# octavian-ganea/equidock_public

Hardware: AMD Instinct MI355X
Metric: protein-pairs/sec (fwd+bwd) per IEGMN stack (higher is better)
Workload: dtype f32; 1 GPU; B: DB5.5-sized batch of 8 pairs x (200,200) residues, k=10, 8-layer IEGMN hdim 64, 50 heads, fp32; pairs_per_gpu=8, nodes_per_gpu=3200, edges_per_gpu=32000, layers=8, parallelism=dp1, weights=PyTorch default init (seed 0), ROT key/query x40 (SURVEY.md section 8c), svd_guard_pairs=0, launch_mode=hipGraph replay

## Files before the change

### equidock_public_amd/_lib.py

```python
import ctypes as C
import os

import torch

HERE = os.path.dirname(os.path.abspath(__file__))
LIB_PATH = os.path.join(HERE, 'libequidock_hip.so')
if os.environ.get('EQD_EXP_LIBRARY'):
    LIB_PATH = os.environ['EQD_EXP_LIBRARY']

EQD_MAX_SRC = 6
ABI_VERSION = 9
PARAMS_PER_LAYER = 19
GLOBAL_PARAMS = 5

c_float_p = C.POINTER(C.c_float)
c_int_p = C.POINTER(C.c_int32)


class EqdGraph(C.Structure):
    _fields_ = [('n_pairs', C.c_int32), ('n_lig', C.c_int32), ('n_rec', C.c_int32), ('n_nodes', C.c_int32),
                ('n_edges', C.c_int32), ('n_tiles', C.c_int32), ('n_att_items', C.c_int32), ('max_seg', C.c_int32),
                ('seg_off', C.c_void_p), ('src', C.c_void_p), ('dst', C.c_void_p), ('rowptr', C.c_void_p),
                ('csc_ptr', C.c_void_p), ('csc_eid', C.c_void_p), ('tile_node', C.c_void_p),
                ('att_items', C.c_void_p), ('res_id', C.c_void_p), ('mu_r_norm', C.c_void_p), ('he', C.c_void_p),
# ... 31 lines not shown
    _fields_ = [('X', C.c_void_p), ('xmask', C.c_void_p), ('ldx', C.c_int32), ('M', C.c_int32), ('Y', C.c_void_p),
                ('ldy', C.c_int32), ('N', C.c_int32), ('rows', C.c_int32), ('out', C.c_void_p), ('o_rs', C.c_int32),
                ('o_cs', C.c_int32), ('bias_out', C.c_void_p), ('slope', C.c_float), ('scale', C.c_float), ('bf16', C.c_int32),
                ('y_bf16', C.c_int32)]


class EqdEdgeParams(C.Structure):
    _fields_ = [('W1', C.c_void_p), ('ldw1', C.c_int32), ('d_in', C.c_int32), ('ln_g', C.c_void_p),
                ('ln_b', C.c_void_p), ('W2', C.c_void_p), ('b2', C.c_void_p), ('Wc1', C.c_void_p),
                ('bc1', C.c_void_p), ('wc2', C.c_void_p), ('bc2', C.c_void_p), ('slope', C.c_float),
                ('ln_eps', C.c_float), ('eta', C.c_float), ('use_dist', C.c_int32), ('use_he', C.c_int32),
                ('bf16', C.c_int32), ('drop_z1', C.c_void_p), ('drop_ch', C.c_void_p), ('drop_scale', C.c_float),
                ('aggr_bf16', C.c_void_p), ('xh_save', C.c_void_p), ('rstd_save', C.c_void_p), ('zpos_save', C.c_void_p)]


class EqdNodeUpdateParams(C.Structure):
    _fields_ = [('d_in', C.c_int32), ('d0', C.c_int32), ('d_out', C.c_int32), ('ld_cross', C.c_int32), ('Wn1', C.c_void_p),
                ('bn1', C.c_void_p), ('ln_g', C.c_void_p), ('ln_b', C.c_void_p), ('Wn2', C.c_void_p), ('bn2', C.c_void_p),
                ('skip_weight_h', C.c_float), ('slope', C.c_float), ('ln_eps', C.c_float), ('bf16', C.c_int32),
                ('drop_mul', C.c_void_p)]


class EqdNodeUpdateGrads(C.Structure):
    _fields_ = [('dWn1', C.c_void_p), ('dbn1', C.c_void_p), ('dln_g', C.c_void_p), ('dln_b', C.c_void_p),
                ('dWn2', C.c_void_p), ('dbn2', C.c_void_p)]


class EqdEdgeGrads(C.Structure):
    _fields_ = [('dW1', C.c_void_p), ('ldw1', C.c_int32), ('db1_unused', C.c_void_p), ('dln_g', C.c_void_p),
                ('dln_b', C.c_void_p), ('dW2', C.c_void_p), ('db2', C.c_void_p), ('dWc1', C.c_void_p),
                ('dbc1', C.c_void_p), ('dwc2', C.c_void_p), ('dbc2', C.c_void_p)]


_lib = None
_is_sim = False
profiling = False


class EquidockHipError(RuntimeError):
    pass


def _declare(lib):
    lib.eqd_abi_version.restype = C.c_int
    lib.eqd_last_error.restype = C.c_char_p
    lib.eqd_tile_edges.restype = C.c_int
    lib.eqd_is_simulator.restype = C.c_int
    lib.eqd_model_saved_bytes.restype = C.c_size_t
    lib.eqd_model_scratch_bytes.restype = C.c_size_t
    lib.eqd_atb_partial_bytes.restype = C.c_size_t
    lib.eqd_edge_message_bwd_workspace_bytes.restype = C.c_size_t
    lib.eqd_keypoint_pool_bwd_workspace_bytes.restype = C.c_size_t
    lib.eqd_clash_workspace_bytes.restype = C.c_size_t
    lib.eqd_node_update_bwd_workspace_bytes.restype = C.c_size_t
    lib.eqd_cross_attention_bwd_ds_workspace_bytes.restype = C.c_size_t
    lib.eqd_profile_name.restype = C.c_char_p
    lib.eqd_profile_us.restype = C.c_float
    lib.eqd_tunables_reload.restype = None
    for name in ('eqd_model_layer_state', 'eqd_model_lrelu_signs', 'eqd_model_head_backward', 'eqd_profile_begin', 'eqd_profile_end', 'eqd_profile_mark', 'eqd_ctx_create', 'eqd_ctx_destroy', 'eqd_model_check', 'eqd_model_forward', 'eqd_model_backward', 'eqd_linear', 'eqd_atb',
                 'eqd_edge_message_fwd', 'eqd_edge_message_bwd', 'eqd_edge_message_bwd_kernel_only',
                 'eqd_cross_attention_fwd', 'eqd_cross_attention_fwd_bf16', 'eqd_cross_attention_bwd_bf16',
                 'eqd_cross_attention_bwd', 'eqd_cross_attention_bwd_ds',
           'eqd_keypoint_pool_fwd', 'eqd_keypoint_pool_bwd', 'eqd_kabsch_fwd', 'eqd_kabsch_bwd',
                 'eqd_rigid_apply_fwd', 'eqd_rigid_apply_bwd', 'eqd_pair_losses_fwd', 'eqd_pair_losses_bwd', 'eqd_scalar_loss', 'eqd_pocket_ot_cost',
                 'eqd_pocket_ot_fwd', 'eqd_pocket_ot_bwd', 'eqd_rigid_augment', 'eqd_protein_graph_distances',
                 'eqd_protein_graph_select', 'eqd_protein_graph_edges', 'eqd_clash_iterations', 'eqd_dropout_pack_edges', 'eqd_dropout_draw',
                 'eqd_node_update_fwd', 'eqd_node_update_bwd', 'eqd_selftest_lane_exchanges'):
        getattr(lib, name).restype = C.c_int


EXPORTS = ('eqd_model_layer_state', 'eqd_model_lrelu_signs', 'eqd_model_head_backward', 'eqd_profile_begin', 'eqd_profile_end', 'eqd_profile_mark', 'eqd_profile_name', 'eqd_profile_us', 'eqd_ctx_create', 'eqd_ctx_destroy', 'eqd_abi_version', 'eqd_last_error', 'eqd_tile_edges', 'eqd_is_simulator', 'eqd_model_saved_bytes', 'eqd_model_saved_layout',
           'eqd_model_scratch_bytes', 'eqd_model_check', 'eqd_model_forward', 'eqd_model_backward', 'eqd_linear',
           'eqd_atb_partial_bytes', 'eqd_atb', 'eqd_edge_message_fwd', 'eqd_edge_message_bwd_workspace_bytes',
           'eqd_edge_message_bwd', 'eqd_edge_message_bwd_kernel_only', 'eqd_cross_attention_fwd',
           'eqd_cross_attention_bwd', 'eqd_cross_attention_bwd_ds', 'eqd_cross_attention_bwd_ds_workspace_bytes', 'eqd_cross_attention_fwd_bf16', 'eqd_cross_attention_bwd_bf16',
           'eqd_keypoint_pool_fwd', 'eqd_keypoint_pool_bwd',
           'eqd_keypoint_pool_bwd_workspace_bytes',
           'eqd_kabsch_fwd', 'eqd_kabsch_bwd', 'eqd_rigid_apply_fwd', 'eqd_rigid_apply_bwd', 'eqd_pair_losses_fwd',
           'eqd_pair_losses_bwd', 'eqd_scalar_loss', 'eqd_pocket_ot_cost', 'eqd_pocket_ot_fwd', 'eqd_pocket_ot_bwd',
           'eqd_rigid_augment', 'eqd_protein_graph_distances', 'eqd_protein_graph_select', 'eqd_protein_graph_edges',
           'eqd_clash_workspace_bytes', 'eqd_clash_iterations', 'eqd_dropout_pack_edges', 'eqd_dropout_draw',
           'eqd_tunables_reload', 'eqd_node_update_fwd', 'eqd_node_update_bwd_workspace_bytes', 'eqd_node_update_bwd',
           'eqd_selftest_lane_exchanges', 'eqd_chain_resident_proj_launches', 'eqd_selftest_node_chain_fwd', 'eqd_model_node_state',
           'eqd_chain_resident_wide_launches', 'eqd_chain_resident_wide_bwd_launches', 'eqd_selftest_node_chain_bwd_wide')


def load_library():
    global _lib, _is_sim
    if _lib is not None:
        return _lib
    if not os.path.exists(LIB_PATH):
        raise EquidockHipError(
            f"{LIB_PATH} is missing: build it with `python -m equidock_public_amd.build` (hipcc, gfx950). "
            "There is no CPU fallback for the IEGMN hot path.")
    lib = C.CDLL(LIB_PATH)
    _declare(lib)
    if lib.eqd_abi_version() != ABI_VERSION:
        raise EquidockHipError(f"ABI version mismatch: library {lib.eqd_abi_version()} != {ABI_VERSION}")
    _lib, _is_sim = lib, bool(lib.eqd_is_simulator())
    return _lib


def load_library_for_testing(path):
    global _lib, _is_sim
    lib = C.CDLL(path)
    _declare(lib)
    _lib, _is_sim = lib, bool(lib.eqd_is_simulator())
    return _lib


def unload_for_testing():
    global _lib, _is_sim
    _lib, _is_sim = None, False


tunables_generation = 0


def reload_tunables():
    global tunables_generation
    tunables_generation += 1
    if _lib is not None:
        _lib.eqd_tunables_reload()


def is_simulator():
    return _is_sim


def check(rc):
    if rc != 0:
        raise EquidockHipError(f"libequidock_hip error {rc}: {_lib.eqd_last_error().decode()}")


def require_device(t, what='tensor'):
    if _is_sim:
        if t.is_cuda:
            raise EquidockHipError(f"{what}: the host simulator only takes CPU tensors")
    elif not t.is_cuda:
        raise EquidockHipError(
            f"{what} is on {t.device}: the IEGMN hot path runs only on an MI355X through libequidock_hip.so "
            "(no CPU fallback)")
    return t


class device_guard:

    def __init__(self, device):
        self._cm = None if (_is_sim or torch.device(device).type != 'cuda') else torch.cuda.device(device)

    def __enter__(self):
        if self._cm is not None:
            self._cm.__enter__()

    def __exit__(self, *exc):
        if self._cm is not None:
            self._cm.__exit__(*exc)
        return False


def ptr(t):
    return C.c_void_p(t.data_ptr()) if t is not None else C.c_void_p(0)


def stream_ptr(device):
    if _is_sim:
        return C.c_void_p(0)
# ... 32 lines not shown
```

### equidock_public_amd/csrc/eqd_attn_fwd_inl.h

```cpp
#pragma once
#include "eqd_common.h"

#ifndef EQD_NATIVE_EXP
#define EQD_NATIVE_EXP(x) __expf(x)
#endif
__device__ __forceinline__ float bwd_exp(float x) { return EQD_NATIVE_EXP(x); }

template <int DB>
struct AttnCfg {
    enum { DS = 16 * DB + 4, KS = 4 * DB, NL = 8 * DB, TILE = 32 * (16 * DB + 4), RED = DB * 2 * 4 * 64 };
};

template <int DB, bool FAST>
struct TileRegs {
    float4 q[FAST ? 8 : 1];
    float4 qx[(FAST && DB > 4) ? 2 : 1];
    f32x4 qv[FAST ? 1 : 2 * DB];
    int nvalid;
};

template <int DB, bool FAST>
__device__ __forceinline__ void tile_load(TileRegs<DB, FAST>& R, const float* __restrict__ M, int d, int r0, int r1,
                                          int lane) {
    int nrows = r1 - r0;
// ... 191 lines not shown
#if !defined(EQD_HOSTSIM) && !defined(EQD_NO_LDS_BATCH)
        __builtin_amdgcn_sched_barrier(0);
#endif
#pragma unroll
        for (int ks = 0; ks < KS; ++ks) {
#pragma unroll
            for (int nb = 0; nb < NB; ++nb) acc[nb] = mfma4(a[ks], F[nb].v[ks], acc[nb]);
        }
    }
}
template <bool BF, int DB, int NB>
__device__ __forceinline__ void mma_r2(f32x4 (&acc)[DB][NB], const float* __restrict__ A, int g, int DS, int l15,
                                       const f32x4 (&B)[2][NB]);
template <bool BF, int DB, int NB>
__device__ __forceinline__ void mma_r(f32x4 (&acc)[DB][NB], const float* __restrict__ A, int row0, int DS, int l15,
                                      const f32x4 (&B)[NB]) {
    if constexpr (BF) {
        s16x4 b[NB];
#pragma unroll
        for (int nb = 0; nb < NB; ++nb) b[nb] = pack_bf4(B[nb][0], B[nb][1], B[nb][2], B[nb][3]);
#pragma unroll
        for (int db = 0; db < DB; ++db) {
            const s16x4 a = pack_bf4(A[row0 * DS + 16 * db + l15], A[(row0 + 1) * DS + 16 * db + l15],
                                     A[(row0 + 2) * DS + 16 * db + l15], A[(row0 + 3) * DS + 16 * db + l15]);
#pragma unroll
            for (int nb = 0; nb < NB; ++nb) acc[db][nb] = mfma_bf(a, b[nb], acc[db][nb]);
        }
    } else {
        float a[4][DB];
#pragma unroll
        for (int r = 0; r < 4; ++r)
#pragma unroll
            for (int db = 0; db < DB; ++db) a[r][db] = A[(row0 + r) * DS + 16 * db + l15];
#if !defined(EQD_HOSTSIM) && !defined(EQD_NO_LDS_BATCH)
        __builtin_amdgcn_sched_barrier(0);
#endif
#pragma unroll
        for (int r = 0; r < 4; ++r)
#pragma unroll
            for (int db = 0; db < DB; ++db) {
#pragma unroll
                for (int nb = 0; nb < NB; ++nb) acc[db][nb] = mfma4(a[r][db], B[nb][r], acc[db][nb]);
            }
    }
}
template <bool BF, int DB, int NB>
__device__ __forceinline__ void mma_r2(f32x4 (&acc)[DB][NB], const float* __restrict__ A, int g, int DS, int l15,
                                       const f32x4 (&B)[2][NB]) {
    if constexpr (BF) {
        s16x8 b[NB];
#pragma unroll
        for (int nb = 0; nb < NB; ++nb)
            b[nb] = cat_bf(pack_bf4(B[0][nb][0], B[0][nb][1], B[0][nb][2], B[0][nb][3]),
                           pack_bf4(B[1][nb][0], B[1][nb][1], B[1][nb][2], B[1][nb][3]));
#pragma unroll
        for (int db = 0; db < DB; ++db) {
            const int r0 = 4 * g, r1 = 16 + 4 * g;
            const s16x8 a = cat_bf(pack_bf4(A[r0 * DS + 16 * db + l15], A[(r0 + 1) * DS + 16 * db + l15],
                                            A[(r0 + 2) * DS + 16 * db + l15], A[(r0 + 3) * DS + 16 * db + l15]),
                                   pack_bf4(A[r1 * DS + 16 * db + l15], A[(r1 + 1) * DS + 16 * db + l15],
                                            A[(r1 + 2) * DS + 16 * db + l15], A[(r1 + 3) * DS + 16 * db + l15]));
#pragma unroll
            for (int nb = 0; nb < NB; ++nb) acc[db][nb] = mfma_bf32(a, b[nb], acc[db][nb]);
        }
    } else {
        mma_r<false, DB, NB>(acc, A, 4 * g, DS, l15, B[0]);
        mma_r<false, DB, NB>(acc, A, 16 + 4 * g, DS, l15, B[1]);
    }
}

template <int DB>
struct alignas(16) AttnFwdSmem {
    typedef AttnCfg<DB> C;
    float Qt[C::TILE];
    float Kt[EQD_WAVES][C::TILE];
    float Vt[EQD_WAVES][C::TILE];
    float sm_m[EQD_WAVES][32], sm_l[EQD_WAVES][32];
    static_assert(C::RED <= C::TILE, "merge buffer must fit a K tile");
};

__device__ __forceinline__ int att_half_item(int b) { return ((b >> 4) << 3) + (b & 7); }
__device__ __forceinline__ int att_half_of(int b) { return (b >> 3) & 1; }

template <int DB, bool FAST, int NB, bool BF = false>
__device__ __forceinline__ void attn_fwd_body(AttnFwdSmem<DB>& sm, const EqdGraph& G, int item, int half, int t, int d,
                                              const float* __restrict__ q, const float* __restrict__ k,
                                              const float* __restrict__ v, float* __restrict__ out,
                                              float* __restrict__ lse, bool group_barriers = false) {
    typedef AttnCfg<DB> C;
    constexpr int DS = C::DS, KS = C::KS;
    float* Qt = sm.Qt;
    float (*Kt)[C::TILE] = sm.Kt;
    float (*Vt)[C::TILE] = sm.Vt;
    float (*sm_m)[32] = sm.sm_m;
    float (*sm_l)[32] = sm.sm_l;
    float (*red)[C::TILE] = Kt;
    const int lane = t & 63, wave = t >> 6;
    const int l15 = lane & 15, g = lane >> 4;
    int b0 = G.att_items[item * 4 + 0], b1 = G.att_items[item * 4 + 1];
    const int o0 = G.att_items[item * 4 + 2], o1 = G.att_items[item * 4 + 3];
    if (NB == 1) {
        b0 += 16 * half;
        b1 = b1 < b0 + 16 ? b1 : b0 + 16;
    }
    if (b0 >= b1) {
        if (group_barriers) {
            static_assert(!(NB == 1) || FAST, "half blocks exist on the float4 path only");
            __syncthreads();
            __syncthreads();
        }
        return;
    }
    int rowq[NB];
    bool qv[NB];
#pragma unroll
    for (int nb = 0; nb < NB; ++nb) {
        rowq[nb] = b0 + 16 * nb + l15;
        qv[nb] = rowq[nb] < b1;
    }

    EQD_TR_WG();
    EQD_TR(0);
    TileRegs<DB, FAST> rk, rv;
    int kt = o0 + 32 * wave;
    tile_load<DB, FAST>(rk, k, d, kt, o1, lane);
    tile_load<DB, FAST>(rv, v, d, kt, o1, lane);
    if (FAST) {
        EQD_TR(1);
        block_tile_stage_fast<DB>(q, DS, b0, b1, Qt, t);
    } else {
        zero_fill(Qt, C::TILE, t, EQD_BLOCK);
        zero_fill(Kt[wave], C::TILE, lane, 64);
        zero_fill(Vt[wave], C::TILE, lane, 64);
        __syncthreads();
        EQD_TR(1);
        block_tile_stage(q, d, DS, b0, b1, Qt, t);
    }
    __syncthreads();
    EQD_TR(2);
    KFrag<BF, KS> qf[NB];
#pragma unroll
    for (int nb = 0; nb < NB; ++nb) kfrag_load<BF, KS>(qf[nb], Qt, 16 * nb + l15, DS, g);

    f32x4 O[DB][NB];
    float mrun[NB], lrun[NB];
#pragma unroll
    for (int nb = 0; nb < NB; ++nb) {
#pragma unroll
        for (int db = 0; db < DB; ++db) O[db][nb] = f4zero();
        mrun[nb] = EQD_NEG_BIG;
        lrun[nb] = 0.f;
    }
    const float* __restrict__ Kw = Kt[wave];
    const float* __restrict__ Vw = Vt[wave];
    EQD_TR(3);
    for (; kt < o1; kt += 32 * EQD_WAVES) {
        wave_lds_fence();
        tile_store<DB, FAST>(rk, Kt[wave], d, lane);
        tile_store<DB, FAST>(rv, Vt[wave], d, lane);
        wave_lds_fence();
        EQD_TR(4);
        tile_load<DB, FAST>(rk, k, d, kt + 32 * EQD_WAVES, o1, lane);
        tile_load<DB, FAST>(rv, v, d, kt + 32 * EQD_WAVES, o1, lane);
        EQD_TR(5);
        f32x4 S[2][NB];
#pragma unroll
        for (int mb = 0; mb < 2; ++mb)
#pragma unroll
            for (int nb = 0; nb < NB; ++nb) S[mb][nb] = f4zero();
#pragma unroll
        for (int mb = 0; mb < 2; ++mb) mma_k<BF, KS, NB>(S[mb], Kw, 16 * mb + l15, DS, g, qf);
        EQD_TR(6);
#pragma unroll
        for (int nb = 0; nb < NB; ++nb) {
            float mx = EQD_NEG_BIG;
#pragma unroll
            for (int mb = 0; mb < 2; ++mb)
#pragma unroll
                for (int r = 0; r < 4; ++r) {
                    const int key = kt + 16 * mb + 4 * g + r;
                    const float sv = BF ? S[mb][nb][r] * 1.44269504088896341f : S[mb][nb][r];
                    const float s = key < o1 ? sv : EQD_NEG_BIG;
                    S[mb][nb][r] = s;
                    mx = fmaxf(mx, s);
                }
            mx = group_max(mx);
            const float mnew = fmaxf(mrun[nb], BF ? ceilf(mx) : mx);
            const float alpha = BF ? exp2_flush(mrun[nb] - mnew) : exp_nooverflow(mrun[nb] - mnew);
            float ps = 0.f;
#pragma unroll
            for (int mb = 0; mb < 2; ++mb)
#pragma unroll
                for (int r = 0; r < 4; ++r) {
                    const int key = kt + 16 * mb + 4 * g + r;
                    const float p = key < o1 ? (BF ? exp2_flush(S[mb][nb][r] - mnew) : exp_nooverflow(S[mb][nb][r] - mnew)) : 0.f;
                    S[mb][nb][r] = p;
                    ps += p;
                }
            lrun[nb] = lrun[nb] * alpha + group_sum(ps);
            mrun[nb] = mnew;
#pragma unroll
            for (int db = 0; db < DB; ++db) O[db][nb] *= alpha;
        }
        EQD_TR(7);
        mma_r2<BF, DB, NB>(O, Vw, g, DS, l15, S);
        EQD_TR(8);
    }
    EQD_TR(9);
    wave_lds_fence();
#pragma unroll
    for (int db = 0; db < DB; ++db)
#pragma unroll
        for (int nb = 0; nb < NB; ++nb)
#pragma unroll
            for (int r = 0; r < 4; ++r) red[wave][((db * 2 + nb) * 4 + r) * 64 + lane] = O[db][nb][r];
    if (g == 0) {
#pragma unroll
        for (int nb = 0; nb < NB; ++nb) {
            sm_m[wave][16 * nb + l15] = mrun[nb];
            sm_l[wave][16 * nb + l15] = lrun[nb];
        }
    }
    __syncthreads();
    float sc[NB][EQD_WAVES], inv[NB], mtot[NB], ltot[NB];
#pragma unroll
    for (int nb = 0; nb < NB; ++nb) {
        float mm = EQD_NEG_BIG;
#pragma unroll
        for (int w = 0; w < EQD_WAVES; ++w) mm = fmaxf(mm, sm_m[w][16 * nb + l15]);
        float ll = 0.f;
#pragma unroll
        for (int w = 0; w < EQD_WAVES; ++w) {
            sc[nb][w] = BF ? exp2_flush(sm_m[w][16 * nb + l15] - mm) : exp_nooverflow(sm_m[w][16 * nb + l15] - mm);
            ll += sm_l[w][16 * nb + l15] * sc[nb][w];
        }
        mtot[nb] = mm;
        ltot[nb] = ll;
        inv[nb] = ll > 0.f ? 1.f / ll : 0.f;
    }
    for (int db = wave; db < DB; db += EQD_WAVES)
#pragma unroll
        for (int nb = 0; nb < NB; ++nb) {
            if (!qv[nb]) continue;
#pragma unroll
            for (int r = 0; r < 4; ++r) {
                float o = 0.f;
#pragma unroll
                for (int w = 0; w < EQD_WAVES; ++w) o += red[w][((db * 2 + nb) * 4 + r) * 64 + lane] * sc[nb][w];
                const int f = 16 * db + 4 * g + r;
                if (f < d) out[(size_t)rowq[nb] * d + f] = o * inv[nb];
            }
        }
    if (wave == 0 && g == 0) {
#pragma unroll
// ... 17 lines not shown
```

### equidock_public_amd/csrc/eqd_edge_kernels.hip

```cpp
#include "eqd_common.h"
#include "eqd_attn_fwd_inl.h"

#include <stdlib.h>
#include <string.h>

#define WS1 45
#define WS2 68
#define TS 68
#define FS 45
#define VEC_LNG 0
#define VEC_LNB 64
#define VEC_B2 128
#define VEC_BC1 192
#define VEC_WC2 256
#define VEC_BC2 320
#define VEC_N 324
#define FWD_WAVES 8
#define BWD_WAVES 8

template <int NW, int TILE_FLOATS>
struct alignas(16) EdgeSmem {
    float w1[64 * WS1];
    float w2[64 * WS2];
    float wc1[64 * WS2];
    float vec[VEC_N];
    float tile[NW][TILE_FLOATS];
};

template <int NW, int TF>
__device__ __forceinline__ void edge_stage_weights(EdgeSmem<NW, TF>& sm, const EqdEdgeParams& P) {
    constexpr int NT = 64 * NW;
    constexpr int N1 = (64 * 11 + NT - 1) / NT, N2 = 1024 / NT;
    const int t = threadIdx.x;
    const int koff = 2 * P.d_in;
    f32x4 v[N1];
    float4 a[N2], b[N2];
    float vec5[5];
#pragma unroll
    for (int j = 0; j < N1; ++j) {
        const int i = t + j * NT;
        const int r = i / 11, c = 4 * (i - r * 11);
        v[j] = ld4u_raw(P.W1 + (size_t)(i < 64 * 11 ? r : 0) * P.ldw1 + koff + c, i < 64 * 11 ? 42 - c : 0, P.W1);
    }
#pragma unroll
    for (int j = 0; j < N2; ++j) {
        const int i = t + j * NT;
        a[j] = ((const float4*)P.W2)[i];
        b[j] = ((const float4*)P.Wc1)[i];
    }
    {
        const int tc = t & 63;
        vec5[0] = P.ln_g[tc];
        vec5[1] = P.ln_b[tc];
        vec5[2] = P.b2[tc];
        vec5[3] = P.bc1[tc];
        vec5[4] = P.wc2[tc];
    }
    const float bc2 = P.bc2[0];
#pragma unroll
    for (int j = 0; j < N1; ++j) {
        const int i = t + j * NT;
        const int r = i / 11, c = 4 * (i - r * 11);
        if (i < 64 * 11) {
            const float4 f = ld4u_fix(v[j], 42 - c);
            float* o = &sm.w1[r * WS1 + c];
            o[0] = f.x;
            if (c + 1 < WS1) o[1] = f.y;
            if (c + 2 < WS1) o[2] = f.z;
            if (c + 3 < WS1) o[3] = f.w;
        }
    }
    if (t < 64) sm.w1[t * WS1 + 44] = 0.f;
#pragma unroll
    for (int j = 0; j < N2; ++j) {
        const int i = t + j * NT;
        const int r = i >> 4, c = (i & 15) * 4;
        *(float4*)&sm.w2[r * WS2 + c] = a[j];
        *(float4*)&sm.wc1[r * WS2 + c] = b[j];
    }
    if (t < 64) {
        sm.vec[VEC_LNG + t] = vec5[0];
        sm.vec[VEC_LNB + t] = vec5[1];
        sm.vec[VEC_B2 + t] = vec5[2];
        sm.vec[VEC_BC1 + t] = vec5[3];
        sm.vec[VEC_WC2 + t] = vec5[4];
    }
    if (t == 0) sm.vec[VEC_BC2] = bc2;
    __syncthreads();
}

__device__ __forceinline__ float rbf_sigma(int k) {
    const float t[16] = {1.f,          1.5f,         2.25f,        3.375f,        5.0625f,     7.59375f,
                         11.390625f,   17.0859375f,  25.62890625f, 38.443359375f, 57.6650390625f,
                         86.49755859375f, 129.746337890625f, 194.6195068359375f, 291.92926025390625f, 1.f};
    return t[k & 15];
}

__device__ __forceinline__ float rbf_neg_inv_sigma(int k) {
    const float t[16] = {-1.f / 1.f,          -1.f / 1.5f,         -1.f / 2.25f,        -1.f / 3.375f,        -1.f / 5.0625f,
                         -1.f / 7.59375f,     -1.f / 11.390625f,   -1.f / 17.0859375f,  -1.f / 25.62890625f,  -1.f / 38.443359375f,
                         -1.f / 57.6650390625f, -1.f / 86.49755859375f, -1.f / 129.746337890625f, -1.f / 194.6195068359375f,
                         -1.f / 291.92926025390625f, -1.f};
    return t[k & 15];
}

template <bool AFF, int NB>
__device__ __forceinline__ void chain64(f32x4 (&out)[4][NB], const f32x4 (&in)[4][NB], const float* __restrict__ W,
                                        const float* __restrict__ ga, const float* __restrict__ be, int l15, int g) {
#pragma unroll
    for (int mbi = 0; mbi < 4; ++mbi) {
        f32x4 b[NB];
#pragma unroll
        for (int nb = 0; nb < NB; ++nb) b[nb] = in[mbi][nb];
        if (AFF) {
// ... 816 lines not shown
        wave_lds_fence();
        EQD_TR(11);
    }
    EQD_TR_WG_END();
}
template <int NW, bool BF, bool DROP = false>
__global__ __launch_bounds__(64 * NW) void k_edge_fwd(EqdGraph G, EqdEdgeParams P, const float* __restrict__ Pn,
                                                              const float* __restrict__ Qn,
                                                              const float* __restrict__ x,
                                                              float* __restrict__ aggr_msg,
                                                              float* __restrict__ x_new) {
    __shared__ EdgeFwdSmem<NW, BF> S;
    edge_fwd_body<NW, BF, DROP>(S, G, P, (int)blockIdx.x, (int)gridDim.x, Pn, Qn, x, aggr_msg, x_new);
}
static int edge_saved_check(const EqdEdgeParams* p, const char* who) {
    const int n = (p->xh_save != nullptr) + (p->rstd_save != nullptr) + (p->zpos_save != nullptr);
    if (n != 0 && n != 3) {
        eqd_set_error("%s: xh_save, rstd_save and zpos_save must all be given or all be NULL", who);
        return EQD_ERR_NULL;
    }
    return EQD_OK;
}
static int edge_drop_mode(const EqdEdgeParams* p, const char* who) {
    if ((p->drop_z1 == nullptr) != (p->drop_ch == nullptr) || (p->drop_z1 && !(p->drop_scale > 0.f))) {
        eqd_set_error("%s: dropout needs both masks (drop_z1, drop_ch) and drop_scale > 0", who);
        return -1;
    }
    return p->drop_z1 ? 1 : 0;
}

union alignas(16) EdgeAttnFwdSmem {
    EdgeFwdSmem<FWD_WAVES, false> edge;
    AttnFwdSmem<4> att[2];
    __device__ EdgeAttnFwdSmem() {}
};
template <bool DROP>
__global__ __launch_bounds__(64 * FWD_WAVES) void k_edge_attn_fwd(EqdGraph G, EqdEdgeParams P, int n_edge,
                                                                   const float* __restrict__ Pn,
                                                                   const float* __restrict__ Qn,
                                                                   const float* __restrict__ x,
                                                                   float* __restrict__ aggr_msg,
                                                                   float* __restrict__ x_new,
                                                                   const float* __restrict__ q,
                                                                   const float* __restrict__ k,
                                                                   const float* __restrict__ v,
                                                                   float* __restrict__ att_out,
                                                                   float* __restrict__ lse) {
    __shared__ EdgeAttnFwdSmem S;
    if ((int)blockIdx.x < n_edge) {
        edge_fwd_body<FWD_WAVES, false, DROP>(S.edge, G, P, (int)blockIdx.x, n_edge, Pn, Qn, x, aggr_msg, x_new);
    } else {
        const int half = (int)threadIdx.x >> 8;
        attn_fwd_body<4, true, 1>(S.att[half], G, (int)blockIdx.x - n_edge, half, (int)threadIdx.x & 255, 64, q, k, v,
                                  att_out, lse, true);
    }
}

union alignas(16) EdgeAttnFwdSmem80 {
    EdgeFwdSmem<FWD_WAVES, false> edge;
    AttnFwdSmem<5> att;
    __device__ EdgeAttnFwdSmem80() {}
};
template <bool DROP>
__global__ __launch_bounds__(64 * FWD_WAVES) void k_edge_attn_fwd80(EqdGraph G, EqdEdgeParams P, int n_edge,
                                                                     const float* __restrict__ Pn,
                                                                     const float* __restrict__ Qn,
                                                                     const float* __restrict__ x,
                                                                     float* __restrict__ aggr_msg,
                                                                     float* __restrict__ x_new,
                                                                     const float* __restrict__ q,
                                                                     const float* __restrict__ k,
                                                                     const float* __restrict__ v,
                                                                     float* __restrict__ att_out,
                                                                     float* __restrict__ lse) {
    __shared__ EdgeAttnFwdSmem80 S;
    if ((int)blockIdx.x < n_edge) {
        edge_fwd_body<FWD_WAVES, false, DROP>(S.edge, G, P, (int)blockIdx.x, n_edge, Pn, Qn, x, aggr_msg, x_new);
    } else {
        if (threadIdx.x >= 256) return;
        attn_fwd_body<5, true, 2>(S.att, G, (int)blockIdx.x - n_edge, 0, (int)threadIdx.x, 80, q, k, v, att_out, lse, false);
    }
}

static int edge_grid(int n_tiles, int waves, int wg_per_cu) {
    if (n_tiles <= 0) return 1;
    const int cus = eqd_num_cus();
    const int slots = cus * waves * wg_per_cu;
    const int rounds = (n_tiles + slots - 1) / slots;
    int blocks = (n_tiles + waves * rounds - 1) / (waves * rounds);
    if (blocks > cus * wg_per_cu) blocks = cus * wg_per_cu;
    return blocks < 1 ? 1 : blocks;
}

extern "C" int eqd_edge_message_fwd(const EqdGraph* g, const EqdEdgeParams* p, const float* P, const float* Q,
                                    const float* x, float* aggr_msg, float* x_new, void* stream) {
    if (!g || !p || !P || !Q || !x || !aggr_msg || !x_new) {
        eqd_set_error("eqd_edge_message_fwd: NULL argument");
        return EQD_ERR_NULL;
    }
    if (g->n_tiles <= 0) return EQD_OK;
    const int blocks = edge_grid(g->n_tiles, FWD_WAVES, 1);
    const int drop = edge_drop_mode(p, "eqd_edge_message_fwd");
    if (drop < 0) return EQD_ERR_NULL;
    if (int rc = edge_saved_check(p, "eqd_edge_message_fwd")) return rc;
    if (p->bf16 && p->use_he && !g->he_bf16) {
        eqd_set_error("eqd_edge_message_fwd: bf16 mode needs EqdGraph.he_bf16");
        return EQD_ERR_NULL;
    }
#define EQD_EDGE_FWD_LAUNCH(BF_, DROP_)                                                                                   \
    hipLaunchKernelGGL(HIP_KERNEL_NAME(k_edge_fwd<FWD_WAVES, BF_, DROP_>), dim3(blocks), dim3(64 * FWD_WAVES), 0,         \
                       (hipStream_t)stream, *g, *p, P, Q, x, aggr_msg, x_new)
    if (p->bf16) {
        if (drop) EQD_EDGE_FWD_LAUNCH(true, true); else EQD_EDGE_FWD_LAUNCH(true, false);
    } else {
        if (drop) EQD_EDGE_FWD_LAUNCH(false, true); else EQD_EDGE_FWD_LAUNCH(false, false);
    }
#undef EQD_EDGE_FWD_LAUNCH
    return eqd_check_launch("k_edge_fwd");
}

int eqd_edge_attn_fused(const EqdGraph* g, const EqdEdgeParams* p, int d_att, const float* q, const float* k, const float* v) {
    if (!eqd_switch_on("EQD_FUSE_FWD")) return 0;
    if (p->bf16 || (d_att != 64 && d_att != 80) || g->n_tiles <= 0 || g->n_att_items <= 0) return 0;
    if (d_att == 80 && !eqd_switch_on("EQD_FUSE_FWD80")) return 0;
    if ((((uintptr_t)q | (uintptr_t)k | (uintptr_t)v) & 15) != 0) return 0;
    const int n_edge = edge_grid(g->n_tiles, FWD_WAVES, 1);
    return n_edge + g->n_att_items <= eqd_num_cus();
}
int eqd_edge_attn_fwd(const EqdGraph* g, const EqdEdgeParams* p, const float* P, const float* Q, const float* x,
                      float* aggr_msg, float* x_new, int d_att, const float* q, const float* k, const float* v,
                      float* att_out, float* lse, hipStream_t st) {
    if (!eqd_edge_attn_fused(g, p, d_att, q, k, v)) {
        int rc = eqd_cross_attention_fwd(g, d_att, q, k, v, att_out, lse, st);
        if (rc) return rc;
        return eqd_edge_message_fwd(g, p, P, Q, x, aggr_msg, x_new, st);
    }
    const int n_edge = edge_grid(g->n_tiles, FWD_WAVES, 1);
    const int drop = edge_drop_mode(p, "eqd_edge_attn_fwd");
    if (drop < 0) return EQD_ERR_NULL;
    if (int rc = edge_saved_check(p, "eqd_edge_attn_fwd")) return rc;
    if (d_att == 80) {
        if (drop)
            hipLaunchKernelGGL(k_edge_attn_fwd80<true>, dim3(n_edge + g->n_att_items), dim3(64 * FWD_WAVES), 0, st, *g, *p, n_edge,
                               P, Q, x, aggr_msg, x_new, q, k, v, att_out, lse);
        else
            hipLaunchKernelGGL(k_edge_attn_fwd80<false>, dim3(n_edge + g->n_att_items), dim3(64 * FWD_WAVES), 0, st, *g, *p, n_edge,
                               P, Q, x, aggr_msg, x_new, q, k, v, att_out, lse);
        return eqd_check_launch("k_edge_attn_fwd");
    }
    if (drop)
        hipLaunchKernelGGL(k_edge_attn_fwd<true>, dim3(n_edge + g->n_att_items), dim3(64 * FWD_WAVES), 0, st, *g, *p, n_edge, P,
                           Q, x, aggr_msg, x_new, q, k, v, att_out, lse);
    else
        hipLaunchKernelGGL(k_edge_attn_fwd<false>, dim3(n_edge + g->n_att_items), dim3(64 * FWD_WAVES), 0, st, *g, *p, n_edge, P,
                           Q, x, aggr_msg, x_new, q, k, v, att_out, lse);
    return eqd_check_launch("k_edge_attn_fwd");
}

#define VP 384
#define V_DLNG 0
#define V_DLNB 64
#define V_DWC2 128
#define V_DBC2 192
#define V_DB2 256
#define V_DBC1 320
#define VA 384
#define WP_W2 0
#define WP_WC1 4096
#define WP_W1 8192
#define WP_N 11264

struct EdgeBwdWs {
    float* dz1;
    float* dxrel;
    float* vecp;
    float* wpart;
};

#define UST 132
__device__ __forceinline__ void slab_store(float* __restrict__ slab, int wave, const f32x4 (&v)[4][1], int l15, int g) {
#pragma unroll
    for (int mb = 0; mb < 4; ++mb)
#pragma unroll
        for (int r = 0; r < 4; ++r) slab[(16 * mb + 4 * g + r) * UST + 16 * wave + l15] = v[mb][0][r];
}
template <int NJ>
__device__ __forceinline__ void slab_atb(f32x4 (&acc)[NJ], const float* __restrict__ Xt, const float* __restrict__ Yt,
                                         int mb, int nb0, int l15, int g) {
#pragma unroll 2
    for (int kc = 0; kc < 8; ++kc) {
        const f32x4 a = *(const f32x4*)&Xt[(16 * mb + l15) * UST + 16 * kc + 4 * g];
        f32x4 b[NJ];
#pragma unroll
        for (int j = 0; j < NJ; ++j) b[j] = *(const f32x4*)&Yt[(16 * (nb0 + j) + l15) * UST + 16 * kc + 4 * g];
#pragma unroll
        for (int u = 0; u < 4; ++u)
#pragma unroll
            for (int j = 0; j < NJ; ++j) acc[j] = mfma4(a[u], b[j][u], acc[j]);
    }
}

__device__ __forceinline__ void feat_atb(f32x4 (&acc)[1], const float* __restrict__ Xt, const float* __restrict__ tiles,
                                         int mb, int nb, int l15, int g) {
    const int c = 16 * nb + l15;
    const bool ok = c < FS;
    const int cc = ok ? c : 0;
#pragma unroll 2
    for (int kc = 0; kc < 8; ++kc) {
        const f32x4 a = *(const f32x4*)&Xt[(16 * mb + l15) * UST + 16 * kc + 4 * g];
        float b[4];
#pragma unroll
        for (int u = 0; u < 4; ++u) b[u] = tiles[kc * (16 * FS) + (4 * g + u) * FS + cc];
#pragma unroll
        for (int u = 0; u < 4; ++u) acc[0] = mfma4(a[u], ok ? b[u] : 0.f, acc[0]);
    }
}

#define USB 72
__device__ __forceinline__ void slab_store_bf(unsigned short* __restrict__ slab, int wave, const f32x4 (&v)[4][1], int l15,
                                              int g) {
#pragma unroll
    for (int mb = 0; mb < 4; ++mb)
        *(s16x4*)&slab[(16 * wave + l15) * USB + 16 * mb + 4 * g] = pack_bf4(v[mb][0][0], v[mb][0][1], v[mb][0][2], v[mb][0][3]);
}
template <int NJ, bool FULL>
__device__ __forceinline__ void slab_atb_bf(f32x4 (&acc)[NJ], const unsigned short* __restrict__ Xr,
                                            const unsigned short* __restrict__ Yr, int mb, int nb0, int l15, int g) {
    const int lo = (4 * g + (l15 >> 2)) * USB + 4 * (l15 & 3);
    const unsigned short* const px = Xr + lo + 16 * mb;
    auto chunk = [&](int kp) {
        const s16x8 a = cat_bf(lds_tr16(px + 32 * kp * USB), lds_tr16(px + (32 * kp + 16) * USB));
#pragma unroll
        for (int j = 0; j < NJ; ++j) {
            const unsigned short* const py = Yr + lo + 16 * (nb0 + j);
            acc[j] = mfma_bf32(a, cat_bf(lds_tr16(py + 32 * kp * USB), lds_tr16(py + (32 * kp + 16) * USB)), acc[j]);
        }
    };
    if constexpr (FULL) {
#pragma unroll
// ... 547 lines not shown
```

### include/equidock_hip.h

```cpp
#ifndef EQUIDOCK_HIP_H
#define EQUIDOCK_HIP_H

#include <stddef.h>
#include <stdint.h>

#ifdef __cplusplus
extern "C" {
#endif

#define EQD_ABI_VERSION 9
#define EQD_TILE_EDGES 32
#define EQD_ATT_BLOCK 32
#define EQD_MAX_SRC 6
#define EQD_PARAMS_PER_LAYER 19
#define EQD_GLOBAL_PARAMS 5

enum {
    EQD_OK = 0,
    EQD_ERR_NULL = 1,
    EQD_ERR_SHAPE = 2,
    EQD_ERR_UNSUPPORTED = 3,
    EQD_ERR_WORKSPACE = 4,
    EQD_ERR_LAUNCH = 5
};
// ... 120 lines not shown
size_t eqd_model_scratch_bytes(const EqdModelDesc* m, const EqdGraph* g);
int eqd_model_saved_layout(const EqdModelDesc* m, const EqdGraph* g);
int eqd_model_check(const EqdModelDesc* m, const EqdGraph* g);

int eqd_model_layer_state(const EqdModelDesc* m, const EqdGraph* g, const void* saved, size_t saved_bytes, int layer,
                          const float** h, int* h_width, const float** x);

int eqd_model_node_state(const EqdModelDesc* m, const EqdGraph* g, const void* saved, size_t saved_bytes, int layer,
                         const float** out , int* d_in, int* d_att);

int eqd_model_lrelu_signs(const EqdModelDesc* m, const EqdGraph* g, const float* const* params, const EqdDropout* drop,
                          const void* saved, size_t saved_bytes, int layer, unsigned char* edge_z1, unsigned char* edge_ch,
                          unsigned char* node, unsigned char* q, unsigned char* k, void* stream);

int eqd_model_forward(const EqdModelDesc* m, const EqdGraph* g, const float* const* params, const EqdDropout* drop,
                      const float* svd_draws,
                      float* lig_out, float* Y_lig, float* Y_rec, float* T, float* b, int32_t* svd_status,
                      void* saved, size_t saved_bytes, void* scratch, size_t scratch_bytes, void* stream, void* ctx);

int eqd_model_backward(const EqdModelDesc* m, const EqdGraph* g, const float* const* params, const EqdDropout* drop,
                       const float* d_lig, const float* d_Ylig, const float* d_Yrec, const float* d_T,
                       const float* d_b, const float* d_h_last, const float* d_x_last,
                       float* grad_flat, const int64_t* grad_offsets,
                       const void* saved, size_t saved_bytes, void* scratch, size_t scratch_bytes, void* stream,
                       void* ctx);

int eqd_model_head_backward(const EqdModelDesc* m, const EqdGraph* g, const float* const* params, const EqdDropout* drop,
                            const float* d_lig, const float* d_Ylig, const float* d_Yrec, const float* d_T,
                            const float* d_b, float* grad_flat, const int64_t* grad_offsets,
                            const void* saved, size_t saved_bytes, void* scratch, size_t scratch_bytes,
                            float* d_h_L, float* d_x_L, void* stream);


typedef struct EqdLinSrc {
    const float* X;
    const float* mask;
    const float* W;
    int32_t ldx, K, w_rs, w_cs;
} EqdLinSrc;
typedef struct EqdLinJob {
    EqdLinSrc s[EQD_MAX_SRC];
    int32_t nsrc, M, act, rows;
    const float* bias;
    const float* ln_g; const float* ln_b; float* pre_ln; int32_t ld_pre;
    const float* R; int32_t ldr;
    float alpha, beta, slope, ln_eps;
    float* Y; int32_t ldy;
    int32_t bf16;
    const float* mul; int32_t ld_mul;
    int32_t pad_to;
    uint16_t* Yb; int32_t ldyb;
} EqdLinJob;
int eqd_linear(const EqdLinJob* jobs , int njobs, void* stream);

typedef struct EqdAtbJob {
    const float* X; const float* xmask; int32_t ldx, M;
    const float* Y; int32_t ldy, N;
    int32_t rows;
    float* out; int32_t o_rs, o_cs;
    float* bias_out;
    float slope;
    float scale;
    int32_t bf16;
    int32_t y_bf16;
} EqdAtbJob;
size_t eqd_atb_partial_bytes(const EqdAtbJob* jobs , int njobs);
int eqd_atb(const EqdAtbJob* jobs , int njobs, void* partial, size_t partial_bytes, void* stream);

typedef struct EqdEdgeParams {
    const float* W1; int32_t ldw1;
    int32_t d_in;
    const float* ln_g; const float* ln_b;
    const float* W2; const float* b2;
    const float* Wc1; const float* bc1; const float* wc2; const float* bc2;
    float slope, ln_eps, eta;
    int32_t use_dist, use_he;
    int32_t bf16;
    const uint32_t* drop_z1; const uint32_t* drop_ch; float drop_scale;
    uint16_t* aggr_bf16;
    float* xh_save; float* rstd_save; uint16_t* zpos_save;
} EqdEdgeParams;
int eqd_edge_message_fwd(const EqdGraph* g, const EqdEdgeParams* p, const float* P, const float* Q,
                         const float* x, float* aggr_msg, float* x_new, void* stream);
typedef struct EqdEdgeGrads {
    float* dW1; int32_t ldw1;
    float* db1_unused;
    float* dln_g; float* dln_b; float* dW2; float* db2; float* dWc1; float* dbc1; float* dwc2; float* dbc2;
} EqdEdgeGrads;
size_t eqd_edge_message_bwd_workspace_bytes(const EqdGraph* g);
int eqd_edge_message_bwd(const EqdGraph* g, const EqdEdgeParams* p, const float* P, const float* Q,
                         const float* x, const float* d_aggr_msg, const float* d_xnew,
                         float* dP, float* dQ, float* dx, const EqdEdgeGrads* grads,
                         void* workspace, size_t ws_bytes, void* stream);

int eqd_edge_message_bwd_kernel_only(const EqdGraph* g, const EqdEdgeParams* p, const float* P, const float* Q,
                                     const float* x, const float* d_aggr_msg, const float* d_xnew,
                                     float* dQ, float* dx, void* workspace, size_t ws_bytes, void* stream);

int eqd_cross_attention_fwd(const EqdGraph* g, int d, const float* q, const float* k, const float* v,
                            float* out, float* lse, void* stream);
int eqd_cross_attention_bwd(const EqdGraph* g, int d, const float* q, const float* k, const float* v,
                            const float* out, const float* lse, const float* d_out,
                            float* dq, float* dk, float* dv, float* delta , void* stream);
size_t eqd_cross_attention_bwd_ds_workspace_bytes(const EqdGraph* g);
int eqd_cross_attention_bwd_ds(const EqdGraph* g, int d, const float* q, const float* k, const float* v,
                               const float* out, const float* lse, const float* d_out,
                               float* dq, float* dk, float* dv, void* ws, size_t ws_bytes, void* stream);

int eqd_cross_attention_fwd_bf16(const EqdGraph* g, int d, const float* q, const float* k, const float* v,
                                 float* out, float* lse, void* stream);
int eqd_cross_attention_bwd_bf16(const EqdGraph* g, int d, const float* q, const float* k, const float* v,
                                 const float* out, const float* lse, const float* d_out,
                                 float* dq, float* dk, float* dv, float* delta, void* stream);

typedef struct EqdNodeUpdateParams {
    int32_t d_in;
    int32_t d0;
    int32_t d_out;
    int32_t ld_cross;
    const float* Wn1;
    const float* bn1;
    const float* ln_g; const float* ln_b;
    const float* Wn2;
    const float* bn2;
    float skip_weight_h, slope, ln_eps;
    int32_t bf16;
    const float* drop_mul;
} EqdNodeUpdateParams;
typedef struct EqdNodeUpdateGrads {
    float* dWn1; float* dbn1; float* dln_g; float* dln_b; float* dWn2; float* dbn2;
} EqdNodeUpdateGrads;
int eqd_node_update_fwd(int rows, const EqdNodeUpdateParams* p, const float* h, const float* aggr_msg,
                        const float* aggr_cross, const float* h0, float* h_out, float* y_act, float* a1n, void* stream);
size_t eqd_node_update_bwd_workspace_bytes(int rows, const EqdNodeUpdateParams* p);
int eqd_node_update_bwd(int rows, const EqdNodeUpdateParams* p, const float* h, const float* aggr_msg,
                        const float* aggr_cross, const float* h0, const float* y_act, const float* a1n,
                        const float* d_h_out, float* d_h, float* d_aggr_msg, float* d_aggr_cross, float* d_h0,
                        const EqdNodeUpdateGrads* grads, void* workspace, size_t ws_bytes, void* stream);

int eqd_keypoint_pool_fwd(const EqdGraph* g, int n_heads, const float* Wk, const float* Wq, const float* qmean,
                          const float* H, const float* Z, float* Y, float* scores, float* lse,
                          float* qp, float* u, void* stream);

size_t eqd_keypoint_pool_bwd_workspace_bytes(const EqdGraph* g, int n_heads);
int eqd_keypoint_pool_bwd(const EqdGraph* g, int n_heads, const float* Wk, const float* Wq, const float* qmean,
                          const float* qp, const float* u, const float* H, const float* Z, const float* scores,
                          const float* lse, const float* dY, float* dH, float* dZ, float* dWk, float* dWq, float* d_hm,
                          void* workspace, size_t ws_bytes, void* stream);

int eqd_kabsch_fwd(int n_pairs, int n_heads, const float* Y, const float* svd_draws, int svd_seed,
                   float* T, float* b, float* A_out, int32_t* status, void* stream);
int eqd_kabsch_bwd(int n_pairs, int n_heads, const float* Y, const float* A, const float* T,
                   const float* dT, const float* db, float* dY, void* stream);

int eqd_rigid_apply_fwd(const EqdGraph* g, const float* T, const float* b, float* lig_out, void* stream);
int eqd_rigid_apply_bwd(const EqdGraph* g, const float* d_lig, float* dT, float* db, void* stream);

int eqd_pair_losses_fwd(const EqdGraph* g, const float* lig_pred, const float* lig_target, const float* rec,
                        float sigma, float surface_ct, float* mse, float* inter, float* s_lig, float* s_rec,
                        void* stream);
int eqd_pair_losses_bwd(const EqdGraph* g, const float* lig_pred, const float* lig_target, const float* rec,
                        float sigma, float surface_ct, const float* s_lig, const float* s_rec, const float* d_mse,
                        const float* d_inter, float* d_lig_pred, void* stream);

int eqd_rigid_augment(const EqdGraph* g, const float* x_lig, const float* R, const float* t, float* new_x,
                      const int32_t* pocket_off, const float* pocket_in, float* pocket_out, void* stream);
// ... 37 lines not shown
```

Measured before the change: 8545 pairs/s.

## Add half-tile edge forward kernel doubling waves per fused edge/attention block

Adds a k_edge_attn_fwd_half kernel that splits each 32-edge tile across two waves of 16 rows each. Twice as many waves run per block, and each wave carries half the register state. Per-node means are then computed cooperatively through LDS, with one half handling channels 0-31 plus coordinate moments and the other channels 32-63. The attention part of the same launch gets a LEAN variant that moves the Q fragment load into the loop and issues the V tile prefetch after the QK MMA behind a sched_barrier, to lower register pressure. The path only runs when the EQD_EDGE_FWD_HALF switch is on, and it adds a launch counter and a selftest entry point.

```diff
diff --git a/equidock_public_amd/_lib.py b/equidock_public_amd/_lib.py
--- a/equidock_public_amd/_lib.py
+++ b/equidock_public_amd/_lib.py
@@ -137,7 +137,8 @@
            'eqd_clash_workspace_bytes', 'eqd_clash_iterations', 'eqd_dropout_pack_edges', 'eqd_dropout_draw',
            'eqd_tunables_reload', 'eqd_node_update_fwd', 'eqd_node_update_bwd_workspace_bytes', 'eqd_node_update_bwd',
            'eqd_selftest_lane_exchanges', 'eqd_chain_resident_proj_launches', 'eqd_selftest_node_chain_fwd', 'eqd_model_node_state',
-           'eqd_chain_resident_wide_launches', 'eqd_chain_resident_wide_bwd_launches', 'eqd_selftest_node_chain_bwd_wide')
+           'eqd_chain_resident_wide_launches', 'eqd_chain_resident_wide_bwd_launches', 'eqd_selftest_node_chain_bwd_wide',
+           'eqd_edge_fwd_half_launches', 'eqd_selftest_edge_attn_fwd')
 
 
 def load_library():
diff --git a/equidock_public_amd/csrc/eqd_attn_fwd_inl.h b/equidock_public_amd/csrc/eqd_attn_fwd_inl.h
--- a/equidock_public_amd/csrc/eqd_attn_fwd_inl.h
+++ b/equidock_public_amd/csrc/eqd_attn_fwd_inl.h
@@ -297,7 +297,7 @@
 __device__ __forceinline__ int att_half_item(int b) { return ((b >> 4) << 3) + (b & 7); }
 __device__ __forceinline__ int att_half_of(int b) { return (b >> 3) & 1; }
 
-template <int DB, bool FAST, int NB, bool BF = false>
+template <int DB, bool FAST, int NB, bool BF = false, bool LEAN = false>
 __device__ __forceinline__ void attn_fwd_body(AttnFwdSmem<DB>& sm, const EqdGraph& G, int item, int half, int t, int d,
                                               const float* __restrict__ q, const float* __restrict__ k,
                                               const float* __restrict__ v, float* __restrict__ out,
@@ -354,8 +354,10 @@
     __syncthreads();
     EQD_TR(2);
     KFrag<BF, KS> qf[NB];
-#pragma unroll
-    for (int nb = 0; nb < NB; ++nb) kfrag_load<BF, KS>(qf[nb], Qt, 16 * nb + l15, DS, g);
+    if constexpr (!LEAN) {
+#pragma unroll
+        for (int nb = 0; nb < NB; ++nb) kfrag_load<BF, KS>(qf[nb], Qt, 16 * nb + l15, DS, g);
+    }
 
     f32x4 O[DB][NB];
     float mrun[NB], lrun[NB];
@@ -376,7 +378,11 @@
         wave_lds_fence();
         EQD_TR(4);
         tile_load<DB, FAST>(rk, k, d, kt + 32 * EQD_WAVES, o1, lane);
-        tile_load<DB, FAST>(rv, v, d, kt + 32 * EQD_WAVES, o1, lane);
+        if constexpr (!LEAN) tile_load<DB, FAST>(rv, v, d, kt + 32 * EQD_WAVES, o1, lane);
+        if constexpr (LEAN) {
+#pragma unroll
+            for (int nb = 0; nb < NB; ++nb) kfrag_load<BF, KS>(qf[nb], Qt, 16 * nb + l15, DS, g);
+        }
         EQD_TR(5);
         f32x4 S[2][NB];
 #pragma unroll
@@ -385,6 +391,12 @@
             for (int nb = 0; nb < NB; ++nb) S[mb][nb] = f4zero();
 #pragma unroll
         for (int mb = 0; mb < 2; ++mb) mma_k<BF, KS, NB>(S[mb], Kw, 16 * mb + l15, DS, g, qf);
+        if constexpr (LEAN) {
+#if !defined(EQD_HOSTSIM)
+            __builtin_amdgcn_sched_barrier(0);
+#endif
+            tile_load<DB, FAST>(rv, v, d, kt + 32 * EQD_WAVES, o1, lane);
+        }
         EQD_TR(6);
 #pragma unroll
         for (int nb = 0; nb < NB; ++nb) {
diff --git a/equidock_public_amd/csrc/eqd_edge_fwd_half_inl.h b/equidock_public_amd/csrc/eqd_edge_fwd_half_inl.h
--- /dev/null
+++ b/equidock_public_amd/csrc/eqd_edge_fwd_half_inl.h
@@ -0,0 +1,137 @@
+#pragma once
+
+#define EDGE_HALF_WAVES (2 * FWD_WAVES)
+#define EDGE_HALF_FEAT1 (32 * TS - 16 * FS)
+static_assert(16 * FS <= 16 * TS && EDGE_HALF_FEAT1 >= 16 * TS, "a half's feature tile lies inside its own message rows");
+
+template <int J0, bool MOM>
+__device__ __forceinline__ void edge_half_means(const float* __restrict__ tile, float* __restrict__ sxw, int rp, float invl,
+                                                int nb0, int nn, int n0, int l15, int g, float* __restrict__ aggr_msg) {
+    const int node = nb0 + l15;
+    const int lo = __shfl(rp, node), hi = __shfl(rp, node + 1);
+    const bool nv = node < nn;
+    f32x4 acc[2], accx = f4zero();
+    acc[0] = acc[1] = f4zero();
+#pragma unroll
+    for (int ks = 0; ks < 8; ++ks) {
+        const int e = 4 * ks + g;
+        const float am = (nv && e >= lo && e < hi) ? 1.f : 0.f;
+#pragma unroll
+        for (int j = 0; j < 2; ++j) acc[j] = mfma4(am, tile[e * TS + 16 * (J0 + j) + l15], acc[j]);
+        if constexpr (MOM) accx = mfma4(am, tile[e * TS + 64 + (l15 & 3)], accx);
+    }
+#pragma unroll
+    for (int r = 0; r < 4; ++r) {
+        const int nd = nb0 + 4 * g + r;
+        const float inv = __shfl(invl, nd);
+        if (nd < nn) {
+#pragma unroll
+            for (int j = 0; j < 2; ++j) aggr_msg[(size_t)(n0 + nd) * 64 + 16 * (J0 + j) + l15] = acc[j][r] * inv;
+            if constexpr (MOM) {
+                if (l15 < 3) sxw[3 * nd + l15] = accx[r] * inv;
+            }
+        }
+    }
+}
+
+template <bool DROP>
+__device__ __forceinline__ void edge_fwd_half_body(EdgeFwdSmem<FWD_WAVES, false>& S_, const EqdGraph& G, const EqdEdgeParams& P,
+                                                   int blk, const float* __restrict__ Pn, const float* __restrict__ Qn,
+                                                   const float* __restrict__ x, float* __restrict__ aggr_msg,
+                                                   float* __restrict__ x_new) {
+    auto& sm = S_.sm;
+    EQD_TR_WG();
+    EQD_TR(0);
+    const int lane = threadIdx.x & 63, wave = threadIdx.x >> 6;
+    const int w = wave & (FWD_WAVES - 1), h = wave >> 3;
+    const int l15 = lane & 15, g = lane >> 4;
+    float* tile = sm.tile[w];
+    float* sxw = S_.sxw[w];
+    const int t = blk * FWD_WAVES + w;
+    const bool live = t < G.n_tiles;
+    int n0 = 0, n1 = 0, e0 = 0, ne = 0;
+    if (live) {
+        n0 = G.tile_node[t];
+        n1 = G.tile_node[t + 1];
+        e0 = G.rowptr[n0];
+        ne = G.rowptr[n1] - e0;
+    }
+    edge_stage_weights<FWD_WAVES, 32 * TS, 64 * EDGE_HALF_WAVES>(sm, P);
+    EQD_TR(1);
+    const int nn = n1 - n0;
+    const size_t xo = (size_t)n0 * 3;
+    const int c0 = lane, c1 = lane + 64;
+    int rp = 0;
+    float x0a = 0.f, xa = 0.f, x0b = 0.f, xb = 0.f;
+    if (live) {
+        rp = G.rowptr[n0 + (lane <= nn ? lane : 0)] - e0;
+        if (h == 0) {
+            x0a = G.x0[xo + (c0 < 3 * nn ? c0 : 0)], xa = x[xo + (c0 < 3 * nn ? c0 : 0)];
+            x0b = G.x0[xo + (c1 < 3 * nn ? c1 : 0)], xb = x[xo + (c1 < 3 * nn ? c1 : 0)];
+        }
+        EdgeTileState<1> S;
+        S.n0 = n0;
+        S.n1 = n1;
+        S.ne = ne - 16 * h;
+        S.ne = S.ne < 0 ? 0 : (S.ne > 16 ? 16 : S.ne);
+        S.e0 = S.ne > 0 ? e0 + 16 * h : e0;
+        const int row = 16 * h + l15;
+        if (S.ne > 0) {
+            f32x4 xh[4][1], m[4][1], ch[4][1];
+            edge_tile_forward<1, DROP, false>(G, P, sm.w1, sm.w2, sm.wc1, sm.vec, tile + h * EDGE_HALF_FEAT1, Pn, Qn, x, lane, S,
+                                              xh, m, ch, nullptr);
+            wave_lds_fence();
+#pragma unroll
+            for (int mb = 0; mb < 4; ++mb)
+                *(float4*)&tile[row * TS + 16 * mb + 4 * g] = make_float4(m[mb][0][0], m[mb][0][1], m[mb][0][2], m[mb][0][3]);
+            if (g == 0) {
+#pragma unroll
+                for (int c = 0; c < 3; ++c) tile[row * TS + 64 + c] = S.xrel[0][c] * S.coef[0];
+                tile[row * TS + 67] = 0.f;
+            }
+        } else {
+#pragma unroll
+            for (int mb = 0; mb < 4; ++mb) *(float4*)&tile[row * TS + 16 * mb + 4 * g] = make_float4(0.f, 0.f, 0.f, 0.f);
+            if (g == 0) *(float4*)&tile[row * TS + 64] = make_float4(0.f, 0.f, 0.f, 0.f);
+        }
+    }
+    EQD_TR(10);
+    __syncthreads();
+    if (live) {
+    const int degl = __shfl(rp, (lane + 1) & 63) - rp;
+    const float invl = (lane < nn && degl > 0) ? 1.f / (float)degl : 0.f;
+    if (h == 0) {
+        for (int nb0 = 0; nb0 < nn; nb0 += 16) edge_half_means<0, true>(tile, sxw, rp, invl, nb0, nn, n0, l15, g, aggr_msg);
+        wave_lds_fence();
+        if (c0 < 3 * nn) x_new[xo + c0] = P.eta * x0a + (1.f - P.eta) * xa + sxw[c0];
+        if (c1 < 3 * nn) x_new[xo + c1] = P.eta * x0b + (1.f - P.eta) * xb + sxw[c1];
+    } else {
+        for (int nb0 = 0; nb0 < nn; nb0 += 16) edge_half_means<2, false>(tile, sxw, rp, invl, nb0, nn, n0, l15, g, aggr_msg);
+    }
+    }
+    EQD_TR(11);
+    EQD_TR_WG_END();
+}
+
+template <bool DROP>
+__global__ __launch_bounds__(64 * EDGE_HALF_WAVES) void k_edge_attn_fwd_half(EqdGraph G, EqdEdgeParams P, int n_edge,
+                                                                              const float* __restrict__ Pn,
+                                                                              const float* __restrict__ Qn,
+                                                                              const float* __restrict__ x,
+                                                                              float* __restrict__ aggr_msg,
+                                                                              float* __restrict__ x_new,
+                                                                              const float* __restrict__ q,
+                                                                              const float* __restrict__ k,
+                                                                              const float* __restrict__ v,
+                                                                              float* __restrict__ att_out,
+                                                                              float* __restrict__ lse) {
+    __shared__ EdgeAttnFwdSmem S;
+    if ((int)blockIdx.x < n_edge) {
+        edge_fwd_half_body<DROP>(S.edge, G, P, (int)blockIdx.x, Pn, Qn, x, aggr_msg, x_new);
+    } else {
+        if (threadIdx.x >= 512) return;
+        const int half = (int)threadIdx.x >> 8;
+        attn_fwd_body<4, true, 1, false, true>(S.att[half], G, (int)blockIdx.x - n_edge, half, (int)threadIdx.x & 255, 64, q, k, v,
+                                  att_out, lse, true);
+    }
+}
diff --git a/equidock_public_amd/csrc/eqd_edge_kernels.hip b/equidock_public_amd/csrc/eqd_edge_kernels.hip
--- a/equidock_public_amd/csrc/eqd_edge_kernels.hip
+++ b/equidock_public_amd/csrc/eqd_edge_kernels.hip
@@ -3,6 +3,7 @@
 
 #include <stdlib.h>
 #include <string.h>
+#include <atomic>
 
 #define WS1 45
 #define WS2 68
@@ -27,9 +28,9 @@
     float tile[NW][TILE_FLOATS];
 };
 
-template <int NW, int TF>
+template <int NW, int TF, int NT = 64 * NW>
 __device__ __forceinline__ void edge_stage_weights(EdgeSmem<NW, TF>& sm, const EqdEdgeParams& P) {
-    constexpr int NT = 64 * NW;
+    static_assert(1024 % NT == 0, "W2 / Wc1 are staged as 1024 float4 in whole rounds of the workgroup");
     constexpr int N1 = (64 * 11 + NT - 1) / NT, N2 = 1024 / NT;
     const int t = threadIdx.x;
     const int koff = 2 * P.d_in;
@@ -1012,6 +1013,8 @@
     }
 }
 
+#include "eqd_edge_fwd_half_inl.h"
+
 static int edge_grid(int n_tiles, int waves, int wg_per_cu) {
     if (n_tiles <= 0) return 1;
     const int cus = eqd_num_cus();
@@ -1048,6 +1051,9 @@
 #undef EQD_EDGE_FWD_LAUNCH
     return eqd_check_launch("k_edge_fwd");
 }
+
+static std::atomic<long long> g_edge_fwd_half_launches{0};
+extern "C" long long eqd_edge_fwd_half_launches(void) { return g_edge_fwd_half_launches.load(); }
 
 int eqd_edge_attn_fused(const EqdGraph* g, const EqdEdgeParams* p, int d_att, const float* q, const float* k, const float* v) {
     if (!eqd_switch_on("EQD_FUSE_FWD")) return 0;
@@ -1078,6 +1084,16 @@
                                P, Q, x, aggr_msg, x_new, q, k, v, att_out, lse);
         return eqd_check_launch("k_edge_attn_fwd");
     }
+    if (eqd_switch_on("EQD_EDGE_FWD_HALF") && g->n_tiles <= FWD_WAVES * n_edge) {
+        if (drop)
+            hipLaunchKernelGGL(k_edge_attn_fwd_half<true>, dim3(n_edge + g->n_att_items), dim3(64 * EDGE_HALF_WAVES), 0, st, *g, *p,
+                               n_edge, P, Q, x, aggr_msg, x_new, q, k, v, att_out, lse);
+        else
+            hipLaunchKernelGGL(k_edge_attn_fwd_half<false>, dim3(n_edge + g->n_att_items), dim3(64 * EDGE_HALF_WAVES), 0, st, *g, *p,
+                               n_edge, P, Q, x, aggr_msg, x_new, q, k, v, att_out, lse);
+        ++g_edge_fwd_half_launches;
+        return eqd_check_launch("k_edge_attn_fwd");
+    }
     if (drop)
         hipLaunchKernelGGL(k_edge_attn_fwd<true>, dim3(n_edge + g->n_att_items), dim3(64 * FWD_WAVES), 0, st, *g, *p, n_edge, P,
                            Q, x, aggr_msg, x_new, q, k, v, att_out, lse);
@@ -1085,6 +1101,16 @@
         hipLaunchKernelGGL(k_edge_attn_fwd<false>, dim3(n_edge + g->n_att_items), dim3(64 * FWD_WAVES), 0, st, *g, *p, n_edge, P,
                            Q, x, aggr_msg, x_new, q, k, v, att_out, lse);
     return eqd_check_launch("k_edge_attn_fwd");
+}
+
+extern "C" int eqd_selftest_edge_attn_fwd(const EqdGraph* g, const EqdEdgeParams* p, const float* P, const float* Q,
+                                          const float* x, float* aggr_msg, float* x_new, int d_att, const float* q,
+                                          const float* k, const float* v, float* att_out, float* lse, void* stream) {
+    if (!g || !p || !P || !Q || !x || !aggr_msg || !x_new || !q || !k || !v || !att_out || !lse) {
+        eqd_set_error("eqd_selftest_edge_attn_fwd: NULL argument");
+        return EQD_ERR_NULL;
+    }
+    return eqd_edge_attn_fwd(g, p, P, Q, x, aggr_msg, x_new, d_att, q, k, v, att_out, lse, (hipStream_t)stream);
 }
 
 #define VP 384
diff --git a/include/equidock_hip.h b/include/equidock_hip.h
--- a/include/equidock_hip.h
+++ b/include/equidock_hip.h
@@ -226,6 +226,10 @@
 } EqdEdgeParams;
 int eqd_edge_message_fwd(const EqdGraph* g, const EqdEdgeParams* p, const float* P, const float* Q,
                          const float* x, float* aggr_msg, float* x_new, void* stream);
+long long eqd_edge_fwd_half_launches(void);
+int eqd_selftest_edge_attn_fwd(const EqdGraph* g, const EqdEdgeParams* p, const float* P, const float* Q, const float* x,
+                               float* aggr_msg, float* x_new, int d_att, const float* q, const float* k, const float* v,
+                               float* att_out, float* lse, void* stream);
 typedef struct EqdEdgeGrads {
     float* dW1; int32_t ldw1;
     float* db1_unused;
```

Result: faster. 8642 pairs/s (median of 6 runs) (+1.1%).
